# kasirershahartau/tissue_image_processing

Measured on AMD Instinct MI355X. Metric: frames/sec end-to-end (2048^2, z=30), higher is better.
Workload: dtype f32(f16x3)

## Files before the change

tissue_image_processing_amd/csrc/tip_unet.hip:

```cpp
#include "tip_internal.h"
#include "tip_unet_conv.h"
#include "tip_unet_first.h"
#include "tip_unet_planes.h"
#include <algorithm>
#include <atomic>
#include <type_traits>

namespace tip {

__global__ void __launch_bounds__(256) k_bias_relu_affine_f32(float *__restrict__ x, const float *__restrict__ bias,
                                                              const float *__restrict__ scale, const float *__restrict__ shift,
                                                              long n4, int C)
{
    const long i = (long)blockIdx.x * blockDim.x + threadIdx.x;
    if (i >= n4) return;
    float4 v = reinterpret_cast<float4 *>(x)[i];
    const int c = (int)((i * 4) % C);
    const float4 b = *reinterpret_cast<const float4 *>(bias + c);
    const float4 s = *reinterpret_cast<const float4 *>(scale + c);
    const float4 t = *reinterpret_cast<const float4 *>(shift + c);
    v.x += b.x; v.y += b.y; v.z += b.z; v.w += b.w;
    v.x = v.x > 0.f ? v.x : 0.f; v.y = v.y > 0.f ? v.y : 0.f; v.z = v.z > 0.f ? v.z : 0.f; v.w = v.w > 0.f ? v.w : 0.f;
    v.x = v.x * s.x + t.x; v.y = v.y * s.y + t.y; v.z = v.z * s.z + t.z; v.w = v.w * s.w + t.w;
    reinterpret_cast<float4 *>(x)[i] = v;
}

template <typename Fn>
static int with_pieces(int planes, int format, Fn &&f)
{
    if (format == 1 && planes == 2) return f(std::integral_constant<int, 2>{}, std::true_type{});
    if (format == 0 && planes == 2) return f(std::integral_constant<int, 2>{}, std::false_type{});
    if (format == 0 && planes == 3) return f(std::integral_constant<int, 3>{}, std::false_type{});
    return TIP_ERR_ARG;
}
static bool pieces_ok(int planes, int format) { return with_pieces(planes, format, [](auto, auto) { return TIP_OK; }) == TIP_OK; }

typedef void (*ConvKernel)(const ConvParams);
struct ConvFlavour {
    int code, npl, th, d, da, spb;
    ConvKernel bf16, f16;
};
template <int CODE, int NPL, int TH, int D, int DA = 1, int SPB = 1>
constexpr ConvFlavour conv_flavour()
{
    ConvKernel f16 = nullptr;
    if constexpr (NPL == 2) f16 = k_unet_conv<NPL, TH, D, DA, SPB, true>;
    return {CODE, NPL, TH, D, DA, SPB, k_unet_conv<NPL, TH, D, DA, SPB, false>, f16};
}
constexpr ConvFlavour CONV_FLAVOURS[] = {
    conv_flavour<0, 2, 8, 2>(),
    conv_flavour<1, 2, 16, 2>(),
    conv_flavour<2, 2, 16, 4>(),
    conv_flavour<3, 3, 8, 2>(),
    conv_flavour<4, 2, 16, 2, 2>(),
    conv_flavour<6, 2, 16, 4, 1, 3>(),
};
constexpr int N_CONV_FLAVOURS = sizeof(CONV_FLAVOURS) / sizeof(CONV_FLAVOURS[0]);

}

using namespace tip;

extern "C" {

int tip_bias_relu_affine_f32_dev(float *x, const float *bias, const float *scale, const float *shift, long n, int c, void *stream)
{
    Ctx &cx = ctx();
    if (!cx.stream) return TIP_ERR_HIP;
    if (!x || !bias || !scale || !shift || n < 0 || c < 4 || (c & 3) || (n % c)) return fail(TIP_ERR_ARG, "bias_relu_affine: bad arguments");
    if (n == 0) return TIP_OK;
    hipStream_t s = (hipStream_t)stream;
    hipLaunchKernelGGL(k_bias_relu_affine_f32, dim3(cdiv(n / 4, 256)), dim3(256), 0, s, x, bias, scale, shift, n / 4, c);
    return launch_check("bias_relu_affine");
}


static __global__ void k_unet_range_fetch(const unsigned *__restrict__ word, int *__restrict__ host) { *host = (int)*word; }

static unsigned *unet_status_word(Ctx &c, hipStream_t s)
{
    if (c.unet_status) return c.unet_status;
    unsigned *w = nullptr;
    int *h = nullptr;
    hipError_t e = hipMalloc(&w, sizeof(unsigned));
    if (e == hipSuccess) e = hipHostMalloc(&h, sizeof(int), hipHostMallocMapped);
    if (e == hipSuccess) e = hipMemsetAsync(w, 0, sizeof(unsigned), s);
    if (e != hipSuccess) {
        if (w) (void)hipFree(w);
        if (h) (void)hipHostFree(h);
        fail(TIP_ERR_HIP, "the U-Net's range word: %s", hipGetErrorString(e));
        return nullptr;
    }
    c.unet_status = w;
    c.unet_status_host = h;
    return w;
}

struct ConvPlan {
    int row;
    int ntiles, nblks, xcd_map;
    size_t lds;
};

static int unet_conv_plan(const tip_unet_conv_desc *d, ConvPlan &pl)
{
    if (!d || !d->in0 || !d->weights || (!d->bias && !d->raw_out) || (!d->out && !d->head_out && !d->raw_out)) return fail(TIP_ERR_ARG, "tip_unet_conv_dev: null pointer");
    if (!pieces_ok(d->planes, d->format)) return fail(TIP_ERR_ARG, "tip_unet_conv_dev: pieces are 2 or 3 planes of bf16 (format 0) or 2 planes of fp16 (format 1)");
    if (d->format == 1 && !(d->acc_scale > 0.f)) return fail(TIP_ERR_ARG, "tip_unet_conv_dev: fp16 pieces come with a positive acc_scale");
    if (d->h < 8 || d->w < UC_TW || d->h % 8 || d->w % UC_TW)
        return fail(TIP_ERR_UNSUPPORTED, "tip_unet_conv_dev: the grid %dx%d is not a multiple of the 8x%d pixel tile", d->h, d->w, UC_TW);
    if (d->c0 < UC_KC || d->c0 % UC_KC || d->c1 < 0 || d->c1 % UC_KC || (d->c1 > 0 && !d->in1) || d->cout < UC_BN || d->cout % UC_BN)
        return fail(TIP_ERR_UNSUPPORTED, "tip_unet_conv_dev: channels (%d + %d -> %d) must be multiples of %d / %d", d->c0, d->c1, d->cout, UC_KC, UC_BN);
    if (d->ntaps < 1 || d->ntaps > 9 || d->sy < 1 || d->sx < 1 || d->oy < 0 || d->ox < 0 ||
        (d->h - 1) * d->sy + d->oy >= d->out_h || (d->w - 1) * d->sx + d->ox >= d->out_w)
        return fail(TIP_ERR_ARG, "tip_unet_conv_dev: bad taps / output mapping");
    if ((d->scale == nullptr) != (d->shift == nullptr)) return fail(TIP_ERR_ARG, "tip_unet_conv_dev: scale and shift come together");
    if (18L * d->w * (d->c0 > d->c1 ? d->c0 : d->c1) * 2 >= (1L << 32) - 65536)
        return fail(TIP_ERR_UNSUPPORTED, "tip_unet_conv_dev: 18 rows of %d pixels x %d channels exceed the 4 GB a buffer resource addresses",
                    d->w, d->c0 > d->c1 ? d->c0 : d->c1);
    for (int t = 0; t < d->ntaps; ++t)
        if (d->dy[t] < -1 || d->dy[t] > 1 || d->dx[t] < -1 || d->dx[t] > 1) return fail(TIP_ERR_ARG, "tip_unet_conv_dev: tap offsets are -1, 0 or 1");
    if (d->head_out && (!d->head_w || !d->head_b || d->cout != UC_BN || !d->scale || d->pool_out || d->sy != 1 || d->sx != 1 || d->oy != 0 || d->ox != 0 ||
                        d->out_h != d->h || d->out_w != d->w))
        return fail(TIP_ERR_ARG, "tip_unet_conv_dev: the fused head needs a 128-channel Conv2D + BatchNorm layer with the plain output mapping");
    if (d->pool_out && (d->sy != 1 || d->sx != 1 || d->oy != 0 || d->ox != 0 || d->out_h != d->h || d->out_w != d->w))
        return fail(TIP_ERR_ARG, "tip_unet_conv_dev: pool_out needs the plain output mapping");
    if (d->raw_out && (d->head_out || d->pool_out)) return fail(TIP_ERR_ARG, "tip_unet_conv_dev: raw output goes without the head and the pooled map");
    if (d->seed && (d->sy != 1 || d->sx != 1 || d->oy != 0 || d->ox != 0 || d->out_h != d->h || d->out_w != d->w))
        return fail(TIP_ERR_ARG, "tip_unet_conv_dev: the accumulator seed needs the plain output mapping");
    const int t8 = tuning().unet_tile8;
    const bool want8 = t8 == 1 || (t8 < 0 && d->ntaps == 9 && d->c0 + d->c1 <= 128);
    const int th = (d->planes == 2 && d->h % 16 == 0 && !want8) ? 16 : 8;
    const int dist = (th == 16 && d->ntaps >= 4) ? 4 : 2;
    const int da = (th == 16 && d->ntaps <= 2) ? 2 : 1;
    const int threads = th * 32, hp = UC_HW * (th + 2);
    pl.ntiles = (d->h / th) * (d->w / UC_TW); pl.nblks = d->cout / UC_BN;
    pl.xcd_map = (tuning().unet_xcd_map && pl.nblks > 1 && pl.ntiles % 8 == 0) ? 1 : 0;
    const int a_per = (d->planes * ((hp * 2 + 63) / 64) * 64 + threads - 1) / threads;
    const int spb = (th == 16 && dist == 4 && d->ntaps == 9 && tuning().unet_spb > 1) ? 3 : 1;
    pl.lds = (size_t)(da + 1) * a_per * threads * 16 + (size_t)(spb > 1 ? 3 * spb : dist + 1) * d->planes * 256 * 16;
    for (pl.row = 0; pl.row < N_CONV_FLAVOURS; ++pl.row) {
        const ConvFlavour &f = CONV_FLAVOURS[pl.row];
        if (f.npl == d->planes && f.th == th && f.d == dist && f.da == da && f.spb == spb) return TIP_OK;
    }
    return fail(TIP_ERR_UNSUPPORTED, "tip_unet_conv_dev: no kernel flavour <%d, %d, %d, %d, %d>", d->planes, th, dist, da, spb);
}

int tip_unet_conv_flavour(const tip_unet_conv_desc *d)
{
    ConvPlan pl;
    const int rc = unet_conv_plan(d, pl);
    return rc ? rc : CONV_FLAVOURS[pl.row].code;
}

int tip_unet_conv_dev(const tip_unet_conv_desc *d, void *stream)
{
    Ctx &c = ctx();
    if (!c.stream) return TIP_ERR_HIP;
    ConvPlan pl;
    if (const int rc = unet_conv_plan(d, pl)) return rc;
    ConvParams p;
    p.in0 = (const uint16_t *)d->in0; p.in1 = (const uint16_t *)(d->c1 > 0 ? d->in1 : d->in0);
    p.c0 = d->c0; p.c1 = d->c1; p.H = d->h; p.W = d->w;
    p.w = (const uint16_t *)d->weights; p.ntaps = d->ntaps;
    for (int t = 0; t < 9; ++t) {
        p.dy[t] = t < d->ntaps ? d->dy[t] : 0; p.dx[t] = t < d->ntaps ? d->dx[t] : 0;
    }
    p.cout = d->cout; p.bias = d->bias; p.scale = d->scale; p.shift = d->shift;
    p.out = (uint16_t *)d->out; p.outH = d->out_h; p.outW = d->out_w; p.sy = d->sy; p.sx = d->sx; p.oy = d->oy; p.ox = d->ox;
    p.pool_out = (uint16_t *)d->pool_out;
    p.acc_scale = d->format == 1 ? d->acc_scale : 1.f;
    p.status = nullptr;
    if (d->format == 1 && !d->raw_out && !(p.status = unet_status_word(c, (hipStream_t)stream))) return TIP_ERR_HIP;
#ifdef UC_TRACE
    static unsigned long long *trace_dev = nullptr;
    if (!trace_dev) { TIP_HIP(hipMalloc(&trace_dev, 1024)); }
    TIP_HIP(hipMemsetAsync(trace_dev, 0, 1024, (hipStream_t)stream));
    p.trace = trace_dev;
#endif
    p.head_w = d->head_w; p.head_b = d->head_b; p.head_out = d->head_out;
    p.raw_out = d->raw_out; p.seed = d->seed;
    p.xcd_map = pl.xcd_map;
    const ConvFlavour &fl = CONV_FLAVOURS[pl.row];
    const ConvKernel kernel = d->format == 1 ? fl.f16 : fl.bf16;
    const int threads = fl.th * 32;
    const size_t lds = pl.lds;
    const dim3 grid = p.xcd_map ? dim3((unsigned)(pl.ntiles * pl.nblks)) : dim3(pl.ntiles, pl.nblks);
    hipStream_t s = (hipStream_t)stream;
    static std::atomic<unsigned> attr_done[64];
    const unsigned bit = 1u << (2 * pl.row + d->format);
    const int dev = c.device >= 0 && c.device < 64 ? c.device : 0;
    if (!(attr_done[dev].load(std::memory_order_acquire) & bit)) {
        TIP_HIP(hipFuncSetAttribute((const void *)kernel, hipFuncAttributeMaxDynamicSharedMemorySize, (int)lds));
        attr_done[dev].fetch_or(bit, std::memory_order_release);
    }
    hipLaunchKernelGGL(kernel, grid, dim3(threads), lds, s, p);
#ifdef UC_TRACE
    {
        unsigned long long tr[128];
        TIP_HIP(hipStreamSynchronize(s));
        TIP_HIP(hipMemcpy(tr, trace_dev, sizeof tr, hipMemcpyDeviceToHost));
        for (int k = 0; k < fl.th / 2; ++k) {
            const unsigned long long *t = tr + 16 * k;
            const double n = (double)t[4];
            fprintf(stderr, "UC_TRACE th %d spb %d taps %d cin %d cout %d grid %dx%d wave %d simd %d: per STEP (shader clocks; sums over the loop / steps): copies %.0f, products %.0f (first MFMA out after %.0f), "
                            "vmcnt wait %.0f, barrier %.0f, total %.0f; steps %.0f; whole loop %.0f, prologue %.0f, epilogue %.0f clocks\n",
                    fl.th, fl.spb, d->ntaps, d->c0 + d->c1, d->cout, d->h, d->w, k, (int)((t[7] >> 4) & 3), t[0] / n, t[2] / n, t[1] / n, t[6] / n, (t[3] - t[6]) / n, t[5] / n, n, (double)t[5], (double)t[8], (double)t[9]);
        }
    }
#endif
    return launch_check("unet_conv");
}

int tip_unet_compose_border_dev(const void *x, int planes, int format, int h, int w, int cin, int cout, const float *row_w, const float *col_w,
                                const float *corner_w, const float *bias_tab, float *part, float xscale, void *stream)
{
    Ctx &c = ctx();
    if (!c.stream) return TIP_ERR_HIP;
    if (!x || !row_w || !col_w || !corner_w || !bias_tab || !part || !pieces_ok(planes, format) ||
        h < 1 || w < 1 || cin < 1 || cout < 128 || cout % 128 || !(xscale > 0.f))
        return fail(TIP_ERR_ARG, "tip_unet_compose_border_dev: bad arguments");
    hipStream_t s = (hipStream_t)stream;
    const int H2 = 2 * h, W2 = 2 * w;
    const long nb = (2L * W2 + 2L * (H2 - 2)) * (cout / 4);
    hipLaunchKernelGGL(k_unet_compose_edge_bias, dim3((unsigned)cdiv(nb, 256)), dim3(256), 0, s, part, H2, W2, cout, bias_tab);
    EdgeParams p;
    p.x = (const uint16_t *)x; p.xplane = (long)h * w * cin; p.planes = planes; p.f16 = format; p.xscale = xscale;
    p.cin = cin; p.cout = cout; p.part = part;
    const long wstride = (long)cin * cout;
    p.L = w; p.x0 = (long)(h - 1) * w * cin; p.xstep = cin; p.tapmask = 0x1f;
    for (int t = 0; t < 5; ++t) p.wgt[t] = row_w + t * wstride;
    p.o0 = (long)(H2 - 1) * W2 * cout; p.ostep = cout;
    hipLaunchKernelGGL(k_unet_compose_edge, dim3((unsigned)cdiv(p.L, EB_J), (unsigned)(cout / EB_CO)), dim3(EB_CO * EB_G), 0, s, p);
    p.L = h; p.x0 = (long)(w - 1) * cin; p.xstep = (long)w * cin;
    for (int t = 0; t < 5; ++t) p.wgt[t] = col_w + t * wstride;
    p.o0 = (long)(W2 - 1) * cout; p.ostep = (long)W2 * cout;
    hipLaunchKernelGGL(k_unet_compose_edge, dim3((unsigned)cdiv(p.L, EB_J), (unsigned)(cout / EB_CO)), dim3(EB_CO * EB_G), 0, s, p);
    p.L = 1; p.x0 = ((long)(h - 1) * w + (w - 1)) * cin; p.xstep = cin; p.tapmask = 0x8;
    for (int t = 0; t < 5; ++t) p.wgt[t] = corner_w;
    p.o0 = ((long)(H2 - 1) * W2 + (W2 - 2)) * cout; p.ostep = cout;
    hipLaunchKernelGGL(k_unet_compose_edge, dim3(1, (unsigned)(cout / EB_CO)), dim3(EB_CO * EB_G), 0, s, p);
    return launch_check("unet_compose_border");
}

int tip_unet_conv_first_dev(const float *in, int h, int w, const float *wgt, const float *bias, const float *scale, const float *shift,
                            void *out, int planes, int format, void *stream)
{
    Ctx &c = ctx();
    if (!c.stream) return TIP_ERR_HIP;
    if (!in || !wgt || !bias || !scale || !shift || !out || h < 1 || w < 1 || w % FIRST_RUN || ((long)h * w) % FIRST_PIX || !pieces_ok(planes, format))
        return fail(TIP_ERR_ARG, "tip_unet_conv_first_dev: bad arguments (w must be a multiple of 32, h * w of 256)");
    const dim3 grid((unsigned)((long)h * w / FIRST_PIX));
    hipStream_t s = (hipStream_t)stream;
    unsigned *status = nullptr;
    if (format == 1 && !(status = unet_status_word(c, s))) return TIP_ERR_HIP;
    return with_pieces(planes, format, [&](auto npl, auto f16) {
        hipLaunchKernelGGL((k_unet_conv_first<decltype(npl)::value, decltype(f16)::value>), grid, dim3(256), 0, s, in, h, w, wgt, bias, scale, shift, (uint16_t *)out, status);
        return launch_check("unet_conv_first");
    });
}

int tip_unet_conv_first_packed_dev(const float *in, int h, int w, const void *packed_weights, float acc_scale, const float *bias,
                                   const float *scale, const float *shift, void *out, void *stream)
{
    Ctx &c = ctx();
    if (!c.stream) return TIP_ERR_HIP;
    if (!in || !packed_weights || !bias || !scale || !shift || !out || h < 1 || w < 1 || w % FIRST_RUN || ((long)h * w) % FIRST_PIX)
        return fail(TIP_ERR_ARG, "tip_unet_conv_first_packed_dev: bad arguments (w must be a multiple of 32, h * w of 256)");
    hipStream_t s = (hipStream_t)stream;
    unsigned *status = unet_status_word(c, s);
    if (!status) return TIP_ERR_HIP;
    const long wgs = (long)h * w / 128;
    const int per_cu = tuning().unet_first_mfma > 1 ? tuning().unet_first_mfma : FIRST_MFMA_WGS_PER_CU;
    const dim3 grid((unsigned)std::min(wgs, 256L * per_cu));
    hipLaunchKernelGGL(k_unet_conv_first_mfma, grid, dim3(256), 0, s, in, h, w, (const uint16_t *)packed_weights, acc_scale, bias, scale, shift,
                       (uint16_t *)out, status);
    return launch_check("unet_conv_first_mfma");
}

int tip_unet_first_mfma(void) { return tuning().unet_first_mfma != 0; }

int tip_unet_range_reset(void *stream)
{
    Ctx &c = ctx();
    if (!c.stream) return TIP_ERR_HIP;
    const bool fresh = !c.unet_status;
    unsigned *w = unet_status_word(c, (hipStream_t)stream);
    if (!w) return TIP_ERR_HIP;
    if (!fresh) TIP_HIP(hipMemsetAsync(w, 0, sizeof(unsigned), (hipStream_t)stream));
    return TIP_OK;
}

int tip_unet_range_read(void *stream, int *flags)
{
    Ctx &c = ctx();
    if (!c.stream) return TIP_ERR_HIP;
    if (!flags) return fail(TIP_ERR_ARG, "tip_unet_range_read: null pointer");
    unsigned *w = unet_status_word(c, (hipStream_t)stream);
    if (!w) return TIP_ERR_HIP;
    int *host_dev = nullptr;
    TIP_HIP(hipHostGetDevicePointer((void **)&host_dev, c.unet_status_host, 0));
    hipLaunchKernelGGL(k_unet_range_fetch, dim3(1), dim3(1), 0, (hipStream_t)stream, (const unsigned *)w, host_dev);
    int rc = launch_check("unet_range_fetch");
    if (rc) return rc;
    TIP_HIP(hipStreamSynchronize((hipStream_t)stream));
    *flags = *(volatile int *)c.unet_status_host;
    return TIP_OK;
}

int tip_unet_pool2_dev(const void *in, int h, int w, int ch, int planes, int format, void *out, void *stream)
{
    Ctx &c = ctx();
    if (!c.stream) return TIP_ERR_HIP;
    if (!in || !out || h < 2 || w < 2 || (h & 1) || (w & 1) || ch < 8 || ch % 8 || !pieces_ok(planes, format))
        return fail(TIP_ERR_ARG, "tip_unet_pool2_dev: bad arguments");
    const long n = (long)(h / 2) * (w / 2) * (ch / 8);
    hipStream_t s = (hipStream_t)stream;
    return with_pieces(planes, format, [&](auto npl, auto f16) {
        hipLaunchKernelGGL((k_unet_pool2<decltype(npl)::value, decltype(f16)::value>), dim3(cdiv(n, 256)), dim3(256), 0, s, (const uint16_t *)in, h, w, ch, (uint16_t *)out);
        return launch_check("unet_pool2");
    });
}

int tip_unet_head_dev(const void *in, long npix, const float *wgt, const float *bias, float *out, int planes, int format, int logits, void *stream)
{
    Ctx &c = ctx();
    if (!c.stream) return TIP_ERR_HIP;
    if (!in || !wgt || !bias || !out || npix < 1 || !pieces_ok(planes, format))
        return fail(TIP_ERR_ARG, "tip_unet_head_dev: bad arguments");
    hipStream_t s = (hipStream_t)stream;
    const dim3 grid(cdiv(npix * 8, 256));
    return with_pieces(planes, format, [&](auto npl, auto f16) {
        hipLaunchKernelGGL((k_unet_head<decltype(npl)::value, decltype(f16)::value>), grid, dim3(256), 0, s, (const uint16_t *)in, npix, wgt, bias, out, logits);
        return launch_check("unet_head");
    });
}

}
```

tissue_image_processing_amd/csrc/tip_unet_conv.h:

```cpp
#pragma once
#include "tip_internal.h"

namespace tip {

typedef __bf16 bf16x8 __attribute__((ext_vector_type(8)));
typedef float f32x16 __attribute__((ext_vector_type(16)));
typedef __bf16 bf16x2 __attribute__((ext_vector_type(2)));
typedef float f32x2 __attribute__((ext_vector_type(2)));
typedef _Float16 f16x8 __attribute__((ext_vector_type(8)));
typedef _Float16 f16x2 __attribute__((ext_vector_type(2)));
constexpr float UC_F16_MAX = 65504.f;

constexpr int UC_TW = 32;
constexpr int UC_BN = 128;
constexpr int UC_KC = 16;
constexpr int UC_HW = UC_TW + 2;

struct ConvParams {
    const uint16_t *in0, *in1;
    int c0, c1;
    int H, W;
    const uint16_t *w;
    int ntaps;
    int dy[9], dx[9];
    int cout;
    const float *bias, *scale, *shift;
    uint16_t *out;
    int outH, outW, sy, sx, oy, ox;
    const float *head_w, *head_b;
    float *head_out;
#ifdef UC_TRACE
    unsigned long long *trace;
#endif
    int xcd_map;
    float acc_scale;
    uint16_t *pool_out;
    float *raw_out;
    const float *seed;
    unsigned *status;
};

__device__ __forceinline__ unsigned bf16_rne_bits(float v)
{
    const unsigned b = __float_as_uint(v);
    return (b + 0x7fffu + ((b >> 16) & 1u)) >> 16;
}
__device__ __forceinline__ float bf16_bits_to_f32(unsigned h) { return __uint_as_float(h << 16); }
__device__ __forceinline__ float relu_bits(float v) { return __int_as_float(max(__float_as_int(v), 0)); }
__device__ __forceinline__ float fmax_raw(float a, float b)
{
    float r;
    asm("v_max_f32 %0, %1, %2" : "=v"(r) : "v"(a), "v"(b));
    return r;
}
__device__ __forceinline__ float fmax_pair(float v)
{
    float r;
    asm("s_nop 1\n\tv_max_f32_dpp %0, %1, %1 quad_perm:[1,0,3,2] row_mask:0xf bank_mask:0xf" : "=v"(r) : "v"(v));
    return r;
}

typedef __attribute__((address_space(3))) unsigned char lds_byte;

template <bool F16>
__device__ __forceinline__ f32x16 uc_mfma(const uint4 &a, const uint4 &b, const f32x16 &c)
{
    if constexpr (F16) return __builtin_amdgcn_mfma_f32_32x32x16_f16(__builtin_bit_cast(f16x8, a), __builtin_bit_cast(f16x8, b), c, 0, 0, 0);
    else return __builtin_amdgcn_mfma_f32_32x32x16_bf16(__builtin_bit_cast(bf16x8, a), __builtin_bit_cast(bf16x8, b), c, 0, 0, 0);
}
template <bool F16>
__device__ __forceinline__ unsigned uc_piece_word(float &a, float &b, bool more)
{
    if constexpr (F16) {
        f16x2 hv;
        hv[0] = (_Float16)a;
        hv[1] = (_Float16)b;
        if (more) {
            a -= (float)hv[0];
            b -= (float)hv[1];
        }
        return __builtin_bit_cast(unsigned, hv);
    } else {
        bf16x2 hv;
        hv[0] = (__bf16)a;
        hv[1] = (__bf16)b;
        const unsigned w = __builtin_bit_cast(unsigned, hv);
        if (more) {
            const f32x2 r = f32x2{a, b} - f32x2{__uint_as_float(w << 16), __uint_as_float(w & 0xffff0000u)};
            a = r[0];
            b = r[1];
        }
        return w;
    }
}
template <bool F16>
__device__ __forceinline__ float uc_piece_value(unsigned halfword)
{
    if constexpr (F16) return (float)__builtin_bit_cast(_Float16, (unsigned short)halfword);
    else return __uint_as_float(halfword << 16);
}
__device__ __forceinline__ float uc_sat_f16(float v) { return __builtin_amdgcn_fmed3f(v, -UC_F16_MAX, UC_F16_MAX); }
__device__ __forceinline__ float uc_amax3(float m, float a, float b)
{
    asm("v_maximum3_f32 %0, %0, |%1|, |%2|" : "+v"(m) : "v"(a), "v"(b));
    return m;
}
__device__ __forceinline__ void uc_range_flag(float amax, unsigned *status, int lane)
{
    if (__any(!(amax <= UC_F16_MAX))) {
        if (lane == 0) atomicOr(status, 1u);
    }
}

template <bool F16>
__device__ __forceinline__ f32x2 uc_biased(const f32x2 &a, const f32x2 &inv2, const f32x2 &b)
{
    if constexpr (F16) return __builtin_elementwise_fma(a, inv2, b);
    else return a + b;
}
template <bool F16>
__device__ __forceinline__ void uc_clamp4(f32x2 &v01, f32x2 &v23, float &amax)
{
    if constexpr (F16) {
        amax = uc_amax3(uc_amax3(amax, v01[0], v01[1]), v23[0], v23[1]);
        v01 = f32x2{uc_sat_f16(v01[0]), uc_sat_f16(v01[1])};
        v23 = f32x2{uc_sat_f16(v23[0]), uc_sat_f16(v23[1])};
    }
}
template <bool F16>
__device__ __forceinline__ void uc_activate4(f32x2 &v01, f32x2 &v23, const float4 &b, const float4 &s, const float4 &t, const f32x2 &inv2, float &amax)
{
    v01 = uc_biased<F16>(v01, inv2, f32x2{b.x, b.y});
    v23 = uc_biased<F16>(v23, inv2, f32x2{b.z, b.w});
    v01 = __builtin_elementwise_fma(f32x2{relu_bits(v01[0]), relu_bits(v01[1])}, f32x2{s.x, s.y}, f32x2{t.x, t.y});
    v23 = __builtin_elementwise_fma(f32x2{relu_bits(v23[0]), relu_bits(v23[1])}, f32x2{s.z, s.w}, f32x2{t.z, t.w});
    uc_clamp4<F16>(v01, v23, amax);
}
template <bool F16>
__device__ __forceinline__ void uc_activate4(f32x2 &v01, f32x2 &v23, const float4 &b, const f32x2 &inv2, float &amax)
{
    v01 = uc_biased<F16>(v01, inv2, f32x2{b.x, b.y});
    v23 = uc_biased<F16>(v23, inv2, f32x2{b.z, b.w});
    uc_clamp4<F16>(v01, v23, amax);
}

template <bool F16>
__device__ __forceinline__ uint4 uc_pack8(float &v0, float &v1, float &v2, float &v3, float &v4, float &v5, float &v6, float &v7, bool more)
{
    uint4 w;
    w.x = uc_piece_word<F16>(v0, v1, more);
    w.y = uc_piece_word<F16>(v2, v3, more);
    w.z = uc_piece_word<F16>(v4, v5, more);
    w.w = uc_piece_word<F16>(v6, v7, more);
    return w;
}

constexpr int EP_ROW = 272, EP_BYTES = 32 * EP_ROW;

__device__ __forceinline__ void uc_softmax2(float z0, float z1, float *out, long i0, long i1)
{
    const float zm = z0 > z1 ? z0 : z1;
    const float e0 = __expf(z0 - zm), e1 = __expf(z1 - zm);
    const float es = e0 + e1;
    out[i0] = e0 / es;
    out[i1] = e1 / es;
}

#ifdef UC_TRACE
__device__ unsigned long long uc_trace_wait_ticks;
template <int N>
__device__ __forceinline__ unsigned long long uc_wait_barrier_timed()
{
    asm volatile("s_waitcnt vmcnt(%0) lgkmcnt(0)" ::"n"(N) : "memory");
    const unsigned long long t = __builtin_amdgcn_s_memtime();
    asm volatile("s_waitcnt lgkmcnt(0)\n\ts_barrier" ::: "memory");
    return t;
}
#endif
template <int N>
__device__ __forceinline__ void uc_wait_barrier()
{
    asm volatile("s_waitcnt vmcnt(%0) lgkmcnt(0)\n\ts_barrier" ::"n"(N) : "memory");
}

template <int NPL, int TH, int D, int DA = 1, int SPB = 1, bool F16 = false>
__global__ void __launch_bounds__(TH * 32, (NPL == 2) ? 2 : 1) k_unet_conv(const ConvParams p)
{
#if defined(__HIP_DEVICE_COMPILE__)
#ifdef UC_TRACE
    const unsigned long long tr_enter = __builtin_amdgcn_s_memtime();
#endif
    static_assert(DA == 1 || (DA == 2 && D == 2), "two-chunk activation prefetch: with the two-step weight schedule");
    static_assert(SPB == 1 || (SPB == 3 && D == 4 && DA == 1 && TH == 16), "several steps per barrier: the 16-row kernel with the four-step weight schedule");
    constexpr bool PAIR = SPB > 1;
    constexpr int UC_NBBUF = PAIR ? 3 * SPB : D + 1;
    constexpr int UC_THREADS = TH * 32, UC_HP = UC_HW * (TH + 2);
    static_assert(TH == 8 || (TH == 16 && NPL == 2), "16-row tiles: two pieces (LDS)");
    constexpr int A_GPP = (UC_HP * 2 + 63) / 64, A_PLANE = A_GPP * 64;
    constexpr int A_PER = (NPL * A_PLANE + UC_THREADS - 1) / UC_THREADS;
    constexpr int A_SLOTS = A_PER * UC_THREADS;
    constexpr int A_BYTES = A_SLOTS * 16;
    constexpr int B_PER = NPL * 256 / UC_THREADS;
    static_assert(B_PER * UC_THREADS == NPL * 256, "weight slots divide evenly");
    constexpr int B_BYTES = NPL * 256 * 16;
    extern __shared__ __attribute__((aligned(16))) unsigned char smem[];
    unsigned char *sA = smem, *sB = smem + (DA + 1) * A_BYTES;
    const int tid = threadIdx.x, lane = tid & 63;
    const int wave = __builtin_amdgcn_readfirstlane(tid >> 6);
    const int tilesX = p.W / UC_TW;
    const int nblks = p.cout / UC_BN;
    int tile, nblk;
    if (p.xcd_map) {
        const int b = blockIdx.x, xcd = b & 7, j = b >> 3;
        tile = (j / nblks) * 8 + xcd;
        nblk = j - (j / nblks) * nblks;
    } else {
        tile = blockIdx.x;
        nblk = blockIdx.y;
    }
    const int ty0 = (tile / tilesX) * TH, tx0 = (tile % tilesX) * UC_TW;
    const int cin = p.c0 + p.c1, nchunks = cin / UC_KC, nsteps = nchunks * p.ntaps;
    const long in_plane0 = (long)p.H * p.W * p.c0, in_plane1 = (long)p.H * p.W * p.c1;
    const int rowbase = ty0 > 0 ? ty0 - 1 : 0;
    const int winrows = min(p.H, ty0 + TH + 1) - rowbase;

    unsigned a_off[A_PER];
    auto plan_a = [&](int C) {
#pragma unroll
        for (int u = 0; u < A_PER; ++u) {
            const int g = u * (UC_THREADS / 64) + wave, pl = g / A_GPP;
            const int rem = (g - pl * A_GPP) * 64 + lane, px = rem >> 1, half = (rem & 1) ^ ((px >> 3) & 1);
            const int hy = px / UC_HW, hx = px - hy * UC_HW;
            const int gy = ty0 + hy - 1, gx = tx0 + hx - 1;
            const bool inside = pl < NPL && rem < UC_HP * 2 && gy >= 0 && gy < p.H && gx >= 0 && gx < p.W;
            a_off[u] = inside ? (unsigned)((((long)(gy - rowbase) * p.W + gx) * C + half * 8) * 2) : 0xffff0000u;
        }
    };
    plan_a(p.c0);
    bool a_second = false;
    constexpr int RSRC_FLAGS = 0x00020000;
    unsigned long long a_win = (unsigned long long)(p.in0 + (long)rowbase * p.W * p.c0), a_plane_bytes = (unsigned long long)in_plane0 * 2;
    int a_rec = (int)(unsigned)((long)winrows * p.W * p.c0 * 2);
    const __amdgpu_buffer_rsrc_t rs_b = __builtin_amdgcn_make_buffer_rsrc((void *)p.w, 0, (int)0xffffffffu, RSRC_FLAGS);
    auto copy_a = [&](int chunk, int buf) {
        const int cbase = chunk * UC_KC;
        const bool second = cbase >= p.c0;
        if (second && !a_second) {
            a_second = true;
            a_win = (unsigned long long)(p.in1 + (long)rowbase * p.W * p.c1);
            a_plane_bytes = (unsigned long long)in_plane1 * 2;
            a_rec = (int)(unsigned)((long)winrows * p.W * p.c1 * 2);
            if (p.c1 != p.c0) plan_a(p.c1);
        }
        const int soff = (second ? cbase - p.c0 : cbase) * 2;
        lds_byte *dst = (lds_byte *)(sA + buf * A_BYTES + wave * 64 * 16);
#pragma unroll
        for (int u = 0; u < A_PER; ++u) {
            const int pl = min((u * (UC_THREADS / 64) + wave) / A_GPP, NPL - 1);
            const unsigned long long base = a_win + (unsigned long long)pl * a_plane_bytes;
            const unsigned lo = __builtin_amdgcn_readfirstlane((unsigned)base), hi = __builtin_amdgcn_readfirstlane((unsigned)(base >> 32));
            const __amdgpu_buffer_rsrc_t rs = __builtin_amdgcn_make_buffer_rsrc((void *)(((unsigned long long)hi << 32) | lo), 0, __builtin_amdgcn_readfirstlane(a_rec), RSRC_FLAGS);
            __builtin_amdgcn_raw_ptr_buffer_load_lds(rs, dst + u * UC_THREADS * 16, 16, a_off[u], soff, 0, 0);
        }
    };
    const int bq = tid & 255;
    const unsigned b_off = (unsigned)(((tid >> 8) * (UC_BN * UC_KC) + (bq >> 1) * UC_KC + (((bq & 1) ^ ((bq >> 4) & 1))) * 8) * 2);
    auto copy_b = [&](int chunk, int tap, int buf) {
        const int soff = ((tap * nchunks + chunk) * nblks + nblk) * (NPL * UC_BN * UC_KC * 2);
        lds_byte *dst = (lds_byte *)(sB + buf * B_BYTES + wave * 64 * 16);
#pragma unroll
        for (int u = 0; u < B_PER; ++u)
            __builtin_amdgcn_raw_ptr_buffer_load_lds(rs_b, dst + u * UC_THREADS * 16, 16, b_off, soff + u * (UC_THREADS / 256) * (UC_BN * UC_KC * 2), 0, 0);
    };

    f32x16 acc[2][4];
#pragma unroll
    for (int m = 0; m < 2; ++m)
#pragma unroll
        for (int n = 0; n < 4; ++n)
#pragma unroll
            for (int i = 0; i < 16; ++i) acc[m][n][i] = 0.f;

    copy_a(0, 0);
    if (DA == 2 && nchunks > 1) copy_a(1, 1);
    for (int s0 = 0; s0 < (PAIR ? 2 * SPB : D) && s0 < nsteps; ++s0) copy_b(s0 / p.ntaps, s0 % p.ntaps, s0);
    if (p.seed) {
        const float up = 1.f / p.acc_scale;
#pragma unroll
        for (int m = 0; m < 2; ++m) {
            const float *sp = p.seed + ((long)(ty0 + wave * 2 + m) * p.W + tx0 + (lane & 31)) * p.cout + nblk * UC_BN + 16 * (lane >> 5);
#pragma unroll
            for (int n = 0; n < 4; ++n)
#pragma unroll
                for (int q = 0; q < 4; ++q) {
                    const float4 v = *reinterpret_cast<const float4 *>(sp + n * 32 + q * 4);
                    acc[m][n][q * 4 + 0] = F16 ? v.x * up : v.x; acc[m][n][q * 4 + 1] = F16 ? v.y * up : v.y;
                    acc[m][n][q * 4 + 2] = F16 ? v.z * up : v.z; acc[m][n][q * 4 + 3] = F16 ? v.w * up : v.w;
                }
        }
    }
    uc_wait_barrier<0>();

    const int r = lane & 31, h = lane >> 5;
    const int b_row = r * 2 + (h ^ ((r >> 3) & 1));
    int step = 0;
    int nc = D / p.ntaps, nt = D % p.ntaps;
    int buf0 = 0, buf2 = D;
    uint4 fa[2][NPL], fb[4][NPL];
#ifdef UC_TRACE
    unsigned long long tr_copy = 0, tr_read = 0, tr_mfma = 0, tr_bar = 0, tr_t0 = __builtin_amdgcn_s_memtime();
    const bool tracing = blockIdx.x == gridDim.x / 2 && blockIdx.y == 0;
    unsigned long long tr_wait = 0, t_w = 0;
#define UC_T(var) const unsigned long long var = __builtin_amdgcn_s_memtime()
#define UC_WB t_w = uc_wait_barrier_timed
#else
#define UC_T(var)
#define UC_WB uc_wait_barrier
#endif
#define UC_PRODUCT(PA, PB)                                                                                      \
    _Pragma("unroll") for (int m = 0; m < 2; ++m) _Pragma("unroll") for (int n = 0; n < 4; ++n)                 \
        acc[m][n] = uc_mfma<F16>(fb[n][PB], fa[m][PA], acc[m][n]);
    auto step_products = [&](int chunk, int tap) {
        const unsigned char *abuf = sA + (chunk % (DA + 1)) * A_BYTES;
        const unsigned char *bbuf = sB + buf0 * B_BYTES;
        const int dy = p.dy[tap], dx = p.dx[tap];
        int aslot[2];
#pragma unroll
        for (int m = 0; m < 2; ++m) {
            const int px = (wave * 2 + m + 1 + dy) * UC_HW + (r + 1 + dx);
            aslot[m] = px * 2 + (h ^ ((px >> 3) & 1));
        }
        auto read_a = [&](int m, int pl) { fa[m][pl] = *reinterpret_cast<const uint4 *>(abuf + (pl * A_PLANE + aslot[m]) * 16); };
        auto read_b = [&](int n, int pl) { fb[n][pl] = *reinterpret_cast<const uint4 *>(bbuf + (pl * 256 + n * 64 + b_row) * 16); };
        if constexpr (NPL == 2) {
            read_a(0, 1); read_a(1, 1);
#pragma unroll
            for (int n = 0; n < 4; ++n) read_b(n, 0);
            __builtin_amdgcn_sched_barrier(0);
            __builtin_amdgcn_s_setprio(1);
            acc[0][0] = uc_mfma<F16>(fb[0][0], fa[0][1], acc[0][0]);
            __builtin_amdgcn_sched_barrier(0);
            read_a(0, 0); read_a(1, 0);
#pragma unroll
            for (int n = 0; n < 4; ++n) read_b(n, 1);
            __builtin_amdgcn_sched_barrier(0);
#pragma unroll
            for (int n = 1; n < 4; ++n) acc[0][n] = uc_mfma<F16>(fb[n][0], fa[0][1], acc[0][n]);
#pragma unroll
            for (int n = 0; n < 4; ++n) acc[1][n] = uc_mfma<F16>(fb[n][0], fa[1][1], acc[1][n]);
            __builtin_amdgcn_sched_barrier(0);
#ifndef UC_TWO_PRODUCTS
            UC_PRODUCT(0, 1)
#endif
            UC_PRODUCT(0, 0)
            __builtin_amdgcn_s_setprio(0);
        } else {
#pragma unroll
            for (int k = 0; k < NPL; ++k) {
#pragma unroll
                for (int m = 0; m < 2; ++m) read_a(m, NPL - 1 - k);
#pragma unroll
                for (int n = 0; n < 4; ++n) read_b(n, k);
            }
            __builtin_amdgcn_s_setprio(1);
            UC_PRODUCT(2, 0) UC_PRODUCT(1, 1) UC_PRODUCT(0, 2)
            UC_PRODUCT(1, 0)
            UC_PRODUCT(0, 1)
            UC_PRODUCT(0, 0)
            __builtin_amdgcn_s_setprio(0);
        }
    };
    if constexpr (PAIR) {
        int c0 = 0, t0 = 0;
        int cb = (2 * SPB) / p.ntaps, tb = (2 * SPB) % p.ntaps;
        int bb = 0;
        int a_issued = 0;
        auto next = [&](int &c, int &t) { if (++t == p.ntaps) { t = 0; ++c; } };
        auto wrapb = [](int b) { return b >= UC_NBBUF ? b - UC_NBBUF : b; };
        for (int s = 0; s < nsteps; s += SPB) {
            UC_T(t_a);
            const bool issue_a = c0 + 1 < nchunks && c0 + 1 > a_issued;
            const int ca = c0 + 1;
            if (issue_a) a_issued = ca;
            const bool issue_b = s + 2 * SPB < nsteps;
            UC_T(t_b);
#pragma unroll
            for (int k = 0; k < SPB; ++k) {
                buf0 = wrapb(bb + k);
                step_products(c0, t0);
                next(c0, t0);
                if (k == 0 && issue_a) copy_a(ca, ca & 1);
                if (issue_b) { copy_b(cb, tb, wrapb(bb + 2 * SPB + k)); next(cb, tb); }
            }
            UC_T(t_c);
            if (issue_b) { if (issue_a) UC_WB<A_PER + SPB * B_PER>(); else UC_WB<SPB * B_PER>(); }
            else { if (issue_a) UC_WB<A_PER>(); else UC_WB<0>(); }
            bb = wrapb(bb + SPB);
#ifdef UC_TRACE
            UC_T(t_d);
            tr_copy += t_b - t_a; tr_mfma += t_c - t_b; tr_bar += t_d - t_c; tr_wait += t_w - t_c;
#endif
        }
    } else
    for (int chunk = 0; chunk < nchunks; ++chunk) {
        for (int tap = 0; tap < p.ntaps; ++tap, ++step) {
            UC_T(t_a);
            const bool issue_a = tap == 0 && chunk + DA < nchunks;
            const bool issue_b = step + D < nsteps;
            UC_T(t_b);
            step_products(chunk, tap);
            if (issue_a) copy_a(chunk + DA, (chunk + DA) % (DA + 1));
            if (issue_b) copy_b(nc, nt, buf2);
            if (++nt == p.ntaps) { nt = 0; ++nc; }
            UC_T(t_c);
            if constexpr (D == 2) {
                const bool need_a_now = DA == 1 && issue_a && p.ntaps == 1;
                if (issue_b) {
                    if (issue_a && !need_a_now) UC_WB<A_PER + B_PER>(); else UC_WB<B_PER>();
                } else {
                    if (issue_a && !need_a_now) UC_WB<A_PER>(); else UC_WB<0>();
                }
            } else {
                const int left = nsteps - (step + 2);
                const int nb = left < 0 ? 0 : (left > D - 1 ? D - 1 : left);
                const bool a_out = tap <= D - 2 && chunk + 1 < nchunks;
#define UC_WAIT_CASE(NB_) case NB_: if (a_out) UC_WB<NB_ * B_PER + A_PER>(); else UC_WB<NB_ * B_PER>(); break;
                switch (nb) {
                    UC_WAIT_CASE(0) UC_WAIT_CASE(1) UC_WAIT_CASE(2)
                    default: if (a_out) UC_WB<(D - 1) * B_PER + A_PER>(); else UC_WB<(D - 1) * B_PER>(); break;
                }
#undef UC_WAIT_CASE
                static_assert(D <= 4, "wait cases cover D <= 4");
            }
            buf0 = buf0 + 1 == UC_NBBUF ? 0 : buf0 + 1;
            buf2 = buf2 + 1 == UC_NBBUF ? 0 : buf2 + 1;
#ifdef UC_TRACE
            UC_T(t_d);
            tr_copy += t_b - t_a; tr_mfma += t_c - t_b; tr_bar += t_d - t_c; tr_wait += t_w - t_c;
#endif
        }
    }
#ifdef UC_TRACE
    if (tracing && p.trace && lane == 0) {
        unsigned long long *tp = p.trace + 16 * wave;
        tp[0] = tr_copy; tp[1] = tr_read; tp[2] = tr_mfma; tp[3] = tr_bar; tp[4] = (unsigned long long)nsteps;
        tp[5] = __builtin_amdgcn_s_memtime() - tr_t0; tp[6] = tr_wait; tp[7] = (unsigned long long)__builtin_amdgcn_s_getreg((31 << 11) | 4);
        tp[8] = tr_t0 - tr_enter;
    }
    const unsigned long long tr_loop_end = __builtin_amdgcn_s_memtime();
#endif
#undef UC_PRODUCT

    static_assert(UC_THREADS / 64 * EP_BYTES <= (DA + 1) * A_BYTES + UC_NBBUF * B_BYTES, "the staging images fit the tile buffers");
    int pxl = lane & 31, hf = lane >> 5;
    asm volatile("" : "+v"(pxl), "+v"(hf));
    unsigned char *ep = smem + wave * EP_BYTES;
    if (p.raw_out) {
#pragma unroll
        for (int m = 0; m < 2; ++m) {
            const int y = ty0 + wave * 2 + m;
            float *op = p.raw_out + ((long)(y * p.sy + p.oy) * p.outW + ((long)(tx0 + pxl) * p.sx + p.ox)) * p.cout + nblk * UC_BN + 16 * hf;
#pragma unroll
            for (int n = 0; n < 4; ++n)
#pragma unroll
                for (int q = 0; q < 4; ++q) {
                    float4 v = {acc[m][n][q * 4 + 0], acc[m][n][q * 4 + 1], acc[m][n][q * 4 + 2], acc[m][n][q * 4 + 3]};
                    if constexpr (F16) { v.x *= p.acc_scale; v.y *= p.acc_scale; v.z *= p.acc_scale; v.w *= p.acc_scale; }
                    *reinterpret_cast<float4 *>(op + n * 32 + q * 4) = v;
                }
        }
        return;
    }
    {
        const float *bip = p.bias + nblk * UC_BN + 16 * hf;
        const float *scp = p.scale + nblk * UC_BN + 16 * hf, *shp = p.shift + nblk * UC_BN + 16 * hf;
        const f32x2 inv2 = {p.acc_scale, p.acc_scale};
        float amax = 0.f;
#pragma unroll
        for (int n = 0; n < 4; ++n) {
#pragma unroll
            for (int q = 0; q < 4; ++q) {
                const float4 b = *reinterpret_cast<const float4 *>(bip + n * 32 + q * 4);
                if (p.scale) {
                    const float4 s = *reinterpret_cast<const float4 *>(scp + n * 32 + q * 4), t = *reinterpret_cast<const float4 *>(shp + n * 32 + q * 4);
#pragma unroll
                    for (int m = 0; m < 2; ++m) {
                        f32x2 v01 = {acc[m][n][q * 4 + 0], acc[m][n][q * 4 + 1]}, v23 = {acc[m][n][q * 4 + 2], acc[m][n][q * 4 + 3]};
                        uc_activate4<F16>(v01, v23, b, s, t, inv2, amax);
                        acc[m][n][q * 4 + 0] = v01[0]; acc[m][n][q * 4 + 1] = v01[1];
                        acc[m][n][q * 4 + 2] = v23[0]; acc[m][n][q * 4 + 3] = v23[1];
                    }
                } else {
#pragma unroll
                    for (int m = 0; m < 2; ++m) {
                        f32x2 v01 = {acc[m][n][q * 4 + 0], acc[m][n][q * 4 + 1]}, v23 = {acc[m][n][q * 4 + 2], acc[m][n][q * 4 + 3]};
                        uc_activate4<F16>(v01, v23, b, inv2, amax);
                        acc[m][n][q * 4 + 0] = v01[0]; acc[m][n][q * 4 + 1] = v01[1];
                        acc[m][n][q * 4 + 2] = v23[0]; acc[m][n][q * 4 + 3] = v23[1];
                    }
                }
            }
            asm volatile("" ::: "memory");
        }
        if constexpr (F16) uc_range_flag(amax, p.status, lane);
    }
    if (p.head_out) {
        float z[2][2] = {{0.f, 0.f}, {0.f, 0.f}};
        const float *hw0 = p.head_w + 16 * hf, *hw1 = p.head_w + UC_BN + 16 * hf;
#pragma unroll
        for (int n = 0; n < 4; ++n)
#pragma unroll
            for (int q = 0; q < 4; ++q) {
                const float4 a4 = *reinterpret_cast<const float4 *>(hw0 + n * 32 + q * 4), b4 = *reinterpret_cast<const float4 *>(hw1 + n * 32 + q * 4);
                const float wa[4] = {a4.x, a4.y, a4.z, a4.w}, wb[4] = {b4.x, b4.y, b4.z, b4.w};
#pragma unroll
                for (int m = 0; m < 2; ++m)
#pragma unroll
                    for (int j = 0; j < 4; ++j) {
                        z[m][0] = __builtin_fmaf(acc[m][n][q * 4 + j], wa[j], z[m][0]);
                        z[m][1] = __builtin_fmaf(acc[m][n][q * 4 + j], wb[j], z[m][1]);
                    }
            }
#pragma unroll
        for (int m = 0; m < 2; ++m)
#pragma unroll
            for (int c = 0; c < 2; ++c) z[m][c] += __shfl_xor(z[m][c], 32, 64);
        const float z0 = (hf ? z[1][0] : z[0][0]) + p.head_b[0], z1 = (hf ? z[1][1] : z[0][1]) + p.head_b[1];
        const float zm = z0 > z1 ? z0 : z1;
        const float e0 = __expf(z0 - zm), e1 = __expf(z1 - zm);
        const float es = e0 + e1;
        const long o = (long)(ty0 + wave * 2 + hf) * p.W + tx0 + pxl;
        p.head_out[o] = e0 / es;
        p.head_out[(long)p.H * p.W + o] = e1 / es;
        return;
    }
    const int rd_row = lane >> 4, rd_col = (lane & 15) * 16;
    const long out_plane = (long)p.outH * p.outW * p.cout;
    if (p.pool_out) {
        const long pool_plane = (long)(p.outH / 2) * (p.outW / 2) * p.cout;
        const bool oddp = pxl & 1;
        float q8[4][8];
#pragma unroll
        for (int n = 0; n < 4; ++n)
#pragma unroll
            for (int i = 0; i < 16; ++i) {
                const float v = fmax_pair(fmax_raw(acc[0][n][i], acc[1][n][i]));
                if (i < 8) q8[n][i] = v; else if (oddp) q8[n][i - 8] = v;
            }
        uint16_t *prow = p.pool_out + ((long)(ty0 / 2 + wave) * (p.outW / 2) + tx0 / 2) * p.cout + nblk * UC_BN + (lane & 15) * 8;
#pragma unroll
        for (int pl = 0; pl < NPL; ++pl) {
#pragma unroll
            for (int n = 0; n < 4; ++n)
                *reinterpret_cast<uint4 *>(ep + (pxl >> 1) * EP_ROW + (n * 32 + 16 * hf + (oddp ? 8 : 0)) * 2) =
                    uc_pack8<F16>(q8[n][0], q8[n][1], q8[n][2], q8[n][3], q8[n][4], q8[n][5], q8[n][6], q8[n][7], pl + 1 < NPL);
#pragma unroll
            for (int it = 0; it < 4; ++it) {
                const int row = it * 4 + rd_row;
                *reinterpret_cast<uint4 *>(prow + pl * pool_plane + (long)row * p.cout) = *reinterpret_cast<const uint4 *>(ep + row * EP_ROW + rd_col);
            }
        }
    }
#pragma unroll
    for (int m = 0; m < 2; ++m) {
        const int y = ty0 + wave * 2 + m;
        uint16_t *orow = p.out + ((long)(y * p.sy + p.oy) * p.outW + ((long)tx0 * p.sx + p.ox)) * p.cout + nblk * UC_BN + (lane & 15) * 8;
#pragma unroll
        for (int pl = 0; pl < NPL; ++pl) {
#pragma unroll
            for (int n = 0; n < 4; ++n)
#pragma unroll
                for (int q = 0; q < 2; ++q) {
                    float v[8];
#pragma unroll
                    for (int j = 0; j < 8; ++j) v[j] = acc[m][n][q * 8 + j];
                    const uint4 w = uc_pack8<F16>(v[0], v[1], v[2], v[3], v[4], v[5], v[6], v[7], pl + 1 < NPL);
                    if (pl + 1 < NPL) {
#pragma unroll
                        for (int j = 0; j < 8; ++j) acc[m][n][q * 8 + j] = v[j];
                    }
                    *reinterpret_cast<uint4 *>(ep + pxl * EP_ROW + (n * 32 + 16 * hf + 8 * q) * 2) = w;
                }
#pragma unroll
            for (int it = 0; it < 8; ++it) {
                const int row = it * 4 + rd_row;
                *reinterpret_cast<uint4 *>(orow + pl * out_plane + (long)row * p.sx * p.cout) = *reinterpret_cast<const uint4 *>(ep + row * EP_ROW + rd_col);
            }
        }
    }
#ifdef UC_TRACE
    if (tracing && p.trace && lane == 0) {
        asm volatile("s_waitcnt vmcnt(0)" ::: "memory");
        p.trace[16 * wave + 9] = __builtin_amdgcn_s_memtime() - tr_loop_end;
    }
#endif
#endif
}

}
```

Baseline: 20.51.

## Issue LDS fragment reads via inline asm with fine-grained lgkmcnt waits

The two-plane conv inner step now issues ds_read_b128 through inline asm with immediate offsets and waits on lgkmcnt per fragment. Each MFMA can then start as soon as its own operands arrive, instead of the compiler inserting a conservative full wait. The three-steps-per-barrier schedule is also extended to 6-tap layers with at least 256 input channels. The hand-counted waits are fragile: the compiler cannot track the asm reads, so any extra LDS op scheduled between them breaks the counts, and the larger SPB layout raises LDS use for those layers.

```diff
diff --git a/tissue_image_processing_amd/csrc/tip_unet.hip b/tissue_image_processing_amd/csrc/tip_unet.hip
--- a/tissue_image_processing_amd/csrc/tip_unet.hip
+++ b/tissue_image_processing_amd/csrc/tip_unet.hip
@@ -137,7 +137,8 @@
     pl.ntiles = (d->h / th) * (d->w / UC_TW); pl.nblks = d->cout / UC_BN;
     pl.xcd_map = (tuning().unet_xcd_map && pl.nblks > 1 && pl.ntiles % 8 == 0) ? 1 : 0;
     const int a_per = (d->planes * ((hp * 2 + 63) / 64) * 64 + threads - 1) / threads;
-    const int spb = (th == 16 && dist == 4 && d->ntaps == 9 && tuning().unet_spb > 1) ? 3 : 1;
+    const bool three = d->ntaps == 9 || (d->ntaps == 6 && d->c0 + d->c1 >= 256);
+    const int spb = (th == 16 && dist == 4 && three && tuning().unet_spb > 1) ? 3 : 1;
     pl.lds = (size_t)(da + 1) * a_per * threads * 16 + (size_t)(spb > 1 ? 3 * spb : dist + 1) * d->planes * 256 * 16;
     for (pl.row = 0; pl.row < N_CONV_FLAVOURS; ++pl.row) {
         const ConvFlavour &f = CONV_FLAVOURS[pl.row];
diff --git a/tissue_image_processing_amd/csrc/tip_unet_conv.h b/tissue_image_processing_amd/csrc/tip_unet_conv.h
--- a/tissue_image_processing_amd/csrc/tip_unet_conv.h
+++ b/tissue_image_processing_amd/csrc/tip_unet_conv.h
@@ -9,6 +9,7 @@
 typedef float f32x2 __attribute__((ext_vector_type(2)));
 typedef _Float16 f16x8 __attribute__((ext_vector_type(8)));
 typedef _Float16 f16x2 __attribute__((ext_vector_type(2)));
+typedef unsigned u32x4 __attribute__((ext_vector_type(4)));
 constexpr float UC_F16_MAX = 65504.f;
 
 constexpr int UC_TW = 32;
@@ -62,9 +63,10 @@
 
 typedef __attribute__((address_space(3))) unsigned char lds_byte;
 
-template <bool F16>
-__device__ __forceinline__ f32x16 uc_mfma(const uint4 &a, const uint4 &b, const f32x16 &c)
-{
+template <bool F16, typename V>
+__device__ __forceinline__ f32x16 uc_mfma(const V &a, const V &b, const f32x16 &c)
+{
+    static_assert(sizeof(V) == 16, "eight 16-bit pieces");
     if constexpr (F16) return __builtin_amdgcn_mfma_f32_32x32x16_f16(__builtin_bit_cast(f16x8, a), __builtin_bit_cast(f16x8, b), c, 0, 0, 0);
     else return __builtin_amdgcn_mfma_f32_32x32x16_bf16(__builtin_bit_cast(bf16x8, a), __builtin_bit_cast(bf16x8, b), c, 0, 0, 0);
 }
@@ -181,6 +183,28 @@
 __device__ __forceinline__ void uc_wait_barrier()
 {
     asm volatile("s_waitcnt vmcnt(%0) lgkmcnt(0)\n\ts_barrier" ::"n"(N) : "memory");
+}
+
+__device__ __forceinline__ unsigned uc_lds_addr(const unsigned char *q) { return (unsigned)(unsigned long long)(const lds_byte *)q; }
+template <int OFF>
+__device__ __forceinline__ void uc_lds_read(u32x4 &v, unsigned addr)
+{
+    asm volatile("ds_read_b128 %0, %1 offset:%2" : "=v"(v) : "v"(addr), "n"(OFF));
+}
+template <int N>
+__device__ __forceinline__ void uc_lds_wait(u32x4 &a)
+{
+    asm volatile("s_waitcnt lgkmcnt(%1)" : "+v"(a) : "n"(N));
+}
+template <int N>
+__device__ __forceinline__ void uc_lds_wait(u32x4 &a, u32x4 &b)
+{
+    asm volatile("s_waitcnt lgkmcnt(%2)" : "+v"(a), "+v"(b) : "n"(N));
+}
+template <int N>
+__device__ __forceinline__ void uc_lds_wait(u32x4 &a, u32x4 &b, u32x4 &c)
+{
+    asm volatile("s_waitcnt lgkmcnt(%3)" : "+v"(a), "+v"(b), "+v"(c) : "n"(N));
 }
 
 template <int NPL, int TH, int D, int DA = 1, int SPB = 1, bool F16 = false>
@@ -306,7 +330,7 @@
     int step = 0;
     int nc = D / p.ntaps, nt = D % p.ntaps;
     int buf0 = 0, buf2 = D;
-    uint4 fa[2][NPL], fb[4][NPL];
+    u32x4 fa[2][NPL], fb[4][NPL];
 #ifdef UC_TRACE
     unsigned long long tr_copy = 0, tr_read = 0, tr_mfma = 0, tr_bar = 0, tr_t0 = __builtin_amdgcn_s_memtime();
     const bool tracing = blockIdx.x == gridDim.x / 2 && blockIdx.y == 0;
@@ -330,27 +354,46 @@
             const int px = (wave * 2 + m + 1 + dy) * UC_HW + (r + 1 + dx);
             aslot[m] = px * 2 + (h ^ ((px >> 3) & 1));
         }
-        auto read_a = [&](int m, int pl) { fa[m][pl] = *reinterpret_cast<const uint4 *>(abuf + (pl * A_PLANE + aslot[m]) * 16); };
-        auto read_b = [&](int n, int pl) { fb[n][pl] = *reinterpret_cast<const uint4 *>(bbuf + (pl * 256 + n * 64 + b_row) * 16); };
+        auto read_a = [&](int m, int pl) { fa[m][pl] = *reinterpret_cast<const u32x4 *>(abuf + (pl * A_PLANE + aslot[m]) * 16); };
+        auto read_b = [&](int n, int pl) { fb[n][pl] = *reinterpret_cast<const u32x4 *>(bbuf + (pl * 256 + n * 64 + b_row) * 16); };
         if constexpr (NPL == 2) {
-            read_a(0, 1); read_a(1, 1);
-#pragma unroll
-            for (int n = 0; n < 4; ++n) read_b(n, 0);
+            const unsigned ra0 = uc_lds_addr(abuf) + aslot[0] * 16, ra1 = uc_lds_addr(abuf) + aslot[1] * 16, rb = uc_lds_addr(bbuf) + b_row * 16;
+            constexpr int AP = A_PLANE * 16, BP = 256 * 16, BN = 64 * 16;
+            uc_lds_read<AP>(fa[0][1], ra0); uc_lds_read<AP>(fa[1][1], ra1);
+            uc_lds_read<0>(fb[0][0], rb); uc_lds_read<BN>(fb[1][0], rb); uc_lds_read<2 * BN>(fb[2][0], rb); uc_lds_read<3 * BN>(fb[3][0], rb);
             __builtin_amdgcn_sched_barrier(0);
             __builtin_amdgcn_s_setprio(1);
+            uc_lds_wait<3>(fa[0][1], fb[0][0]);
             acc[0][0] = uc_mfma<F16>(fb[0][0], fa[0][1], acc[0][0]);
             __builtin_amdgcn_sched_barrier(0);
-            read_a(0, 0); read_a(1, 0);
-#pragma unroll
-            for (int n = 0; n < 4; ++n) read_b(n, 1);
+            uc_lds_read<0>(fa[0][0], ra0); uc_lds_read<0>(fa[1][0], ra1);
+            uc_lds_read<BP>(fb[0][1], rb); uc_lds_read<BP + BN>(fb[1][1], rb); uc_lds_read<BP + 2 * BN>(fb[2][1], rb); uc_lds_read<BP + 3 * BN>(fb[3][1], rb);
             __builtin_amdgcn_sched_barrier(0);
-#pragma unroll
-            for (int n = 1; n < 4; ++n) acc[0][n] = uc_mfma<F16>(fb[n][0], fa[0][1], acc[0][n]);
+            uc_lds_wait<8>(fb[1][0]);
+            acc[0][1] = uc_mfma<F16>(fb[1][0], fa[0][1], acc[0][1]);
+            uc_lds_wait<7>(fb[2][0]);
+            acc[0][2] = uc_mfma<F16>(fb[2][0], fa[0][1], acc[0][2]);
+            uc_lds_wait<6>(fb[3][0], fa[1][1]);
+            acc[0][3] = uc_mfma<F16>(fb[3][0], fa[0][1], acc[0][3]);
 #pragma unroll
             for (int n = 0; n < 4; ++n) acc[1][n] = uc_mfma<F16>(fb[n][0], fa[1][1], acc[1][n]);
             __builtin_amdgcn_sched_barrier(0);
 #ifndef UC_TWO_PRODUCTS
-            UC_PRODUCT(0, 1)
+            uc_lds_wait<3>(fa[0][0], fa[1][0], fb[0][1]);
+            acc[0][0] = uc_mfma<F16>(fb[0][1], fa[0][0], acc[0][0]);
+            __builtin_amdgcn_sched_barrier(0);
+            uc_lds_wait<2>(fb[1][1]);
+            acc[0][1] = uc_mfma<F16>(fb[1][1], fa[0][0], acc[0][1]);
+            __builtin_amdgcn_sched_barrier(0);
+            uc_lds_wait<1>(fb[2][1]);
+            acc[0][2] = uc_mfma<F16>(fb[2][1], fa[0][0], acc[0][2]);
+            __builtin_amdgcn_sched_barrier(0);
+            uc_lds_wait<0>(fb[3][1]);
+            acc[0][3] = uc_mfma<F16>(fb[3][1], fa[0][0], acc[0][3]);
+#pragma unroll
+            for (int n = 0; n < 4; ++n) acc[1][n] = uc_mfma<F16>(fb[n][1], fa[1][0], acc[1][n]);
+#else
+            uc_lds_wait<0>(fa[0][0], fa[1][0]);
 #endif
             UC_PRODUCT(0, 0)
             __builtin_amdgcn_s_setprio(0);
```

Measured after the change: 20.92, median of 6. 1.02x the previous value.
